# xuyuan/waymo_2d_tracking

Measured on AMD Instinct MI355X. Metric: end-to-end frames/sec (detect+SORT) on 1920x1280 Waymo frames, higher is better.
Workload: dtype f32; 1 GPU; Cascade R-CNN X152-32x8d-FPN dconv (random-init, fp32, batch 1) on synthetic 1920x1280x3 frames -> top-100 detections/frame -> SORT (max_age 2, min_hits 0, all boxes tracked; trackers resident for the whole segment); 5 cameras x 2 frames per step per GPU; 1x1 and dense 3x3 convolutions: f32 operands as exact 3 x bf16 splits, six cross terms on the bf16 matrix cores, f32 accumulate (csrc/det_gemm_s; stage=e2e, parallelism=sequence-shard x1

## Files before the change

include/waymodet.h:

```cpp
#ifndef WAYMODET_H
#define WAYMODET_H
#include <stddef.h>
#include <stdint.h>
#ifdef __cplusplus
extern "C" {
#endif

int wd_roi_pool_fpn_f32(const float* const* feats, const int32_t* heights, const int32_t* widths,
                        const float* scales, int n_levels, int channels, int batch,
                        const float* rois, int n_rois, int pooled, int min_level, int canonical_level,
                        float canonical_size, float* out, void* stream);

size_t wd_nms_workspace(int n);
int wd_select_kept(const uint8_t* keep_mask, const uint8_t* valid, const int64_t* order, int n, int cap, int64_t* out_idx,
                   int32_t* count, void* stream);
int wd_nms_sorted_f32(const float* boxes, const int32_t* idxs, int n, float iou_threshold,
                      uint8_t* keep_mask, int32_t* n_keep, void* workspace, size_t workspace_bytes, void* stream);

size_t wd_gemm_nt_workspace(int M, int N, int K);
int wd_gemm_nt_ws_f32(const float* A, const float* Bt, const float* bias, const float* residual, int relu, int M, int N, int K,
                      float* C, void* workspace, size_t workspace_bytes, void* stream);

int wd_gemm_lt_f32(const float* a, const float* w, const float* bias, const float* residual, float* out, int m, int n, int k,
                   int relu, void* workspace, size_t workspace_bytes, void* stream);
// ... 6 lines not shown
    void* dst;
    long s_n, s_c, s_kh, s_kw;
    long first_block;
    int N, K, C, ksize, flip, reserved;
} WdSplitPackDesc;
int wd_gemm_split_pack_batch(const WdSplitPackDesc* descs_device, int count, long total_blocks, void* stream);
size_t wd_gemm_split_workspace(long M, int N, int K);
int wd_gemm_split_f32(const float* a, long lda, const void* packed_w, const float* bias, const float* residual, float* out, long ldc,
                      int M, int N, int K, int relu, void* workspace, size_t workspace_bytes, void* stream);
int wd_conv_split_f32(const float* x, int batch, int H, int W, int C, const void* packed_w, int ksize, int stride, int pad, const float* bias,
                      const float* residual, float* out, int N, int relu, void* workspace, size_t workspace_bytes, void* stream);
int wd_gemm_split_supported(const float* a, long lda, const float* bias, const float* residual, const float* out, long ldc, long M, int N, int K);
int wd_conv_split_position_major(int batch, int H, int W, int ksize, int stride, int pad);
typedef struct WdSplitIO {
    const float* a;
    long lda;
    const void* a_planes;
    const float* residual;
    const void* residual_planes;
    float* out;
    void* out_planes;
    long ldc;
} WdSplitIO;
size_t wd_split_planes_bytes(long M, int K);
int wd_split_planes_pack_f32(const float* a, long lda, long M, int K, void* planes, void* stream);
int wd_split_planes_unpack_f32(const void* planes, long M, int K, float* out, long ldo, void* stream);
int wd_gemm_split_io(const WdSplitIO* io, const void* packed_w, const float* bias, int M, int N, int K, int relu, void* workspace,
                     size_t workspace_bytes, void* stream);
int wd_nms_segmented_f32(const float* boxes, const int32_t* idxs, const int32_t* seg_offsets, int n_seg, float iou_threshold,
                         uint8_t* keep_mask, int32_t* n_keep, void* workspace, size_t workspace_bytes, void* stream);

size_t wd_rpn_topk_workspace(const int* n_per_level, int n_levels, int k);
int wd_rpn_topk_decode_f32(const float* const* logits, const float* const* deltas, const float* const* anchors,
                           const int* n_per_level, int n_levels, int k, float img_h, float img_w, float scale_clamp,
                           float* out_boxes, float* out_scores, int32_t* out_group, uint8_t* out_valid, void* workspace,
                           size_t workspace_bytes, void* stream);
int wd_sort_candidates_f32(const float* boxes, const float* scores, const int32_t* group, const uint8_t* valid,
                           const uint8_t* valid2 , int n, float* out_boxes, float* out_scores, int32_t* out_group, uint8_t* out_valid, int64_t* out_order,
                           void* stream);
int wd_box_candidates_f32(const float* boxes, const float* s0, const float* s1, const float* s2, const int32_t* n_valid, int rows,
                          int num_classes, float score_thresh, float img_h, float img_w, float* out_boxes, float* out_scores,
                          int32_t* out_group, uint8_t* out_valid, int64_t* out_order, void* stream);
int wd_gather_kept_f32(const uint8_t* keep, const uint8_t* valid, const float* boxes, const float* scores, const int64_t* order,
                       int n, int cap, int num_classes, float* out_boxes, float* out_scores, int64_t* out_class, int32_t* count,
                       void* stream);
int wd_detections_to_wire(const float* boxes, const float* scores, const int64_t* classes, const int32_t* count, int n, int in_w,
                          int in_h, int hflip, int out_w, int out_h, double* xywhs, int32_t* category, void* stream);

size_t wd_deform_packed_weight_floats(int c_in, int c_out, int groups);
int wd_deform_pack_weight(const float* weight_oihw, int c_in, int c_out, int groups, float* packed, void* stream);
const char* wd_deform_conv3x3_variant(int c_in, int groups, int stride, int pad, int has_offset);
const char* wd_deform_conv3x3_last_kernel(void);
int wd_deform_conv3x3_f32(const float* x, const float* offset, const float* mask, const float* packed_weight,
                          const float* scale, const float* bias, int relu,
                          int batch, int h, int w, int c_in, int c_out, int groups, int stride, int pad,
                          float* y, void* stream);
int wd_deform_conv3x3_hint_f32(const float* x, const float* offset, const float* mask, const float* packed_weight,
                               const float* scale, const float* bias, int relu, int batch, int h, int w, int c_in,
                               int c_out, int groups, int stride, int pad, int far_offsets, float* y, void* stream);
size_t wd_deform_table_bytes(int batch, int h, int w);
int wd_deform_offsets_table_f32(const float* partial, int ld, const float* bias, int batch, int h, int w, float* offsets,
                                void* table, void* stream);
int wd_deform_conv3x3_tab_f32(const float* x, const float* offset, const float* mask, const float* packed_weight,
                              const float* scale, const float* bias, int relu, int batch, int h, int w, int c_in,
                              int c_out, int groups, int stride, int pad, int far_offsets, const void* table, float* y,
                              void* stream);

int wd_gemm_nt_f32(const float* A, const float* Bt, const float* bias, const float* residual, int relu,
                   int M, int N, int K, float* C, void* stream);

int wd_groupnorm_relu_nhwc_f32(float* x, const float* gamma, const float* beta, int n, int hw, int c, int groups,
                               float eps, int relu, void* stream);
int wd_groupnorm_relu_out_nhwc_f32(const float* x, float* y, const float* gamma, const float* beta, int n, int hw, int c, int groups,
                                   float eps, int relu, void* stream);
int wd_groupnorm_relu_bwd_nhwc_f32(const float* x, const float* dy, const float* gamma, const float* beta, int n, int hw, int c, int groups,
                                   float eps, int relu, float* dx, float* dgamma, float* dbeta, void* stream);

#define WD_LAYOUT_NCHW_F32 0
#define WD_LAYOUT_NHWC_U8 1
int wd_preprocess_out_shape(int h, int w, double scale, int divisor, int* ho, int* wo, int* hp, int* wp);
int wd_preprocess_f32(const void* src, int src_layout, int batch, int h, int w, double scale, int hflip, int vflip,
                      int swap_rb, const float* mean3, const float* std3, int divisor, float* out, void* stream);

int wd_decode_boxes_f32(const float* deltas, const float* boxes, const int64_t* index, int n, float wx, float wy, float ww,
                        float wh, float scale_clamp, float clip_w, float clip_h, float* out, void* stream);

int wd_roi_pool_fpn_bwd_f32(float* const* grad_feats, const int32_t* heights, const int32_t* widths, const float* scales,
                            int n_levels, int channels, int batch, const float* rois, int n_rois, int pooled, int min_level,
                            int canonical_level, float canonical_size, const float* grad_out, void* stream);
int wd_deform_im2col_f32(const float* x, const float* offset, int batch, int h, int w, int c, int groups, int stride, int pad,
                         float* col, void* stream);
int wd_deform_col2im_f32(const float* dcol, const float* x, const float* offset, int batch, int h, int w, int c, int groups,
                         int stride, int pad, float* dx, float* doffset, void* stream);
size_t wd_deform_bwd_tables_bytes(int batch, int h, int w, int stride);
int wd_deform_dxoff_f32(const float* x, const float* offset, const float* dy, const float* y_act, const float* scale, const float* weight, int batch,
                        int h, int w, int c, int groups, int stride, unsigned char* tables, float* packed_weight, float* dx, float* doffset,
                        void* stream);
size_t wd_deform_dw_scratch_floats(int batch, int h, int w, int c, int groups, int stride);
int wd_deform_dw_f32(const float* x, const float* offset, const float* dy, const float* y_act, const float* scale, int batch, int h, int w, int c,
                     int groups, int stride, float* scratch, float* dw, void* stream);

int wd_tap_shift_add_f32(const float* partial, int ld, int n_out, const float* bias, int batch, int h, int w, int stride,
                         float* out, void* stream);

int wd_upsample2x_nhwc_f32(const float* src, int batch, int h, int w, int c, float* dst, void* stream);

int wd_bias_relu_f32(float* y, const float* bias, long m, int n, int relu, void* stream);

int wd_act_bwd_f32(const float* dy, const float* y, const float* scale, long m, int n, int relu, float* g, void* stream);

int wd_autocontrast_u8(uint8_t* img, int h, int w, void* workspace24, void* stream);

int wd_jpeg_info(const uint8_t* data, int64_t n, int32_t* width, int32_t* height, int32_t* components, int32_t* h_samp,
                 int32_t* v_samp, int32_t* restart_interval);
int wd_jpeg_decode_rgb_u8(const uint8_t* data, int64_t n, uint8_t* rgb, int64_t capacity, int32_t* width, int32_t* height,
                          int32_t* sync_rounds, void* stream);
int wd_jpeg_last_stats(int32_t* out4);

#ifdef __cplusplus
}
#endif
#endif
```

waymo_2d_tracking_amd/build.py:

```python
import os
import subprocess
import sys
from concurrent.futures import ThreadPoolExecutor

HERE = os.path.dirname(os.path.abspath(__file__))
CSRC = os.path.join(HERE, 'csrc')
LIB = os.path.join(CSRC, 'libwaymotrack.so')
HIPCC = os.environ.get('HIPCC', '/opt/rocm/bin/hipcc')
ARCH = 'gfx950'

COMMON = ['--offload-arch=' + ARCH, '-O3', '-std=c++17', '-fPIC', '-fno-fast-math', '-Wall', '-Wno-unused-function']
COMMON += os.environ.get('WD_HIPCC_FLAGS', '').split()
UNITS = {
    'api.hip': [],
    'json_io.hip': [],
    'waymo_proto.hip': [],
    'ensemble.hip': ['-ffp-contract=off'],
    'ensemble_wbf.hip': ['-ffp-contract=off'],
    'sort_engine.hip': ['-ffp-contract=off'],
    'sort_single.hip': ['-ffp-contract=off'],
    'mot_eval.hip': ['-ffp-contract=off'],
    'mot_identity.hip': ['-ffp-contract=off'],
    'mot_hota.hip': ['-ffp-contract=off'],
    'track_refine.hip': ['-ffp-contract=off'],
    'det_eval.hip': ['-ffp-contract=off'],
    'det_roialign.hip': [],
    'det_nms.hip': [],
    'det_deform.hip': [],
    'det_deform_pp.hip': ['-fno-slp-vectorize'],
    'det_gconv.hip': [],
    'det_gemm.hip': ['-munsafe-fp-atomics'],
    'det_gemm_lt.hip': [],
    'det_gemm_split.hip': [],
    'det_misc.hip': [],
    'det_preprocess.hip': ['-ffp-contract=off'],
    'jpeg_decode.hip': [],
    'det_tail.hip': ['-ffp-contract=off'],
    'det_backward.hip': ['-munsafe-fp-atomics'],
    'det_deform_bwd.hip': ['-munsafe-fp-atomics'],
}
DEBUG_UNITS = {'det_gemm_split.hip': [], 'debug/debug_kernels.hip': []}
DEBUG_LIB = os.path.join(CSRC, 'libwaymotrack_debug.so')


def _newer(target, sources):
    if not os.path.exists(target):
        return True
    t = os.path.getmtime(target)
    return any(os.path.getmtime(s) > t for s in sources)


def build(force=False, verbose=True):
    headers = [os.path.join(CSRC, f) for f in os.listdir(CSRC) if f.endswith('.h')]
    headers += [os.path.join(HERE, '..', 'include', f) for f in os.listdir(os.path.join(HERE, '..', 'include'))]
    units = [u for u in UNITS if os.path.exists(os.path.join(CSRC, u))]
    objs = []
    jobs = []
    for u in units:
        src = os.path.join(CSRC, u)
        obj = os.path.join(CSRC, os.path.basename(u).replace('.hip', '.o'))
        objs.append(obj)
        if force or _newer(obj, [src] + headers):
            jobs.append([HIPCC] + COMMON + UNITS[u] + ['-c', src, '-o', obj])

    def run(cmd):
        if verbose:
            print(' '.join(cmd), flush=True)
        r = subprocess.run(cmd, capture_output=True, text=True)
        if r.returncode != 0:
            raise RuntimeError('hipcc failed:\n%s\n%s' % (' '.join(cmd), r.stderr[-6000:]))
        if verbose and r.stderr.strip():
            print(r.stderr[-3000:])
        return 0

    if jobs:
        with ThreadPoolExecutor(max_workers=min(6, len(jobs))) as ex:
            list(ex.map(run, jobs))
    if jobs or force or _newer(LIB, objs):
        run([HIPCC, '--offload-arch=' + ARCH, '-shared', '-fPIC', '-o', LIB] + objs)
    return LIB


def build_debug(force=False, verbose=True):
    build(force, verbose)
    headers = [os.path.join(CSRC, f) for f in os.listdir(CSRC) if f.endswith('.h')] + [os.path.join(CSRC, 'debug', 'waymodet_debug.h')]
    headers += [os.path.join(HERE, '..', 'include', f) for f in os.listdir(os.path.join(HERE, '..', 'include'))]
    objs = [os.path.join(CSRC, os.path.basename(u).replace('.hip', '.o')) for u in UNITS if u not in DEBUG_UNITS]
    jobs = []
    for u, flags in DEBUG_UNITS.items():
        src, obj = os.path.join(CSRC, u), os.path.join(CSRC, os.path.basename(u).replace('.hip', '.dbg.o'))
        objs.append(obj)
        if force or _newer(obj, [src] + headers):
            jobs.append([HIPCC] + COMMON + ['-DWD_DEBUG=1'] + UNITS.get(u, []) + flags + ['-c', src, '-o', obj])
    for cmd in jobs:
        if verbose:
            print(' '.join(cmd), flush=True)
        r = subprocess.run(cmd, capture_output=True, text=True)
        if r.returncode != 0:
            raise RuntimeError('hipcc failed:\n%s\n%s' % (' '.join(cmd), r.stderr[-6000:]))
    if jobs or force or _newer(DEBUG_LIB, objs):
        r = subprocess.run([HIPCC, '--offload-arch=' + ARCH, '-shared', '-fPIC', '-o', DEBUG_LIB] + objs, capture_output=True, text=True)
        if r.returncode != 0:
            raise RuntimeError('link failed:\n%s' % r.stderr[-6000:])
    return DEBUG_LIB


if __name__ == '__main__':
    if os.environ.get('WD_DEBUG_BUILD') == '1':
        print(build_debug(force='--force' in sys.argv))
    else:
        build(force='--force' in sys.argv)
    print(LIB)
```

waymo_2d_tracking_amd/detnet/nn/cascade_rcnn.py:

```python
import math
import os

import torch
from torch import nn
import torch.nn.functional as F

from . import ops

BLOCKS = (3, 8, 36, 3)
STAGE_CH = (256, 512, 1024, 2048)
GROUPS = 32
PIXEL_MEAN = (103.530, 116.280, 123.675)
PIXEL_STD = (57.375, 57.120, 58.395)
SCALE_CLAMP = math.log(1000.0 / 16)


FUSED_TRAINING_EPILOGUES = True


SPLIT_GEMM = os.environ.get('WD_SPLIT_GEMM', '1') != '0'


OFFSET_SPLIT_MIN_ROWS = 30000


SPLIT_PLANES = os.environ.get('WD_SPLIT_PLANES', '0') == '1'
SPLIT_PLANES_MIN_CH = int(os.environ.get('WD_SPLIT_PLANES_MIN_CH', '1024'))


class PlanesAct:

    def __init__(self, planes, n, h, w, c):
        self.planes, self.n, self.h, self.w, self.c = planes, n, h, w, c


DECISION_LOG = None


def _split_ok(cin, cout):
    return SPLIT_GEMM and cin % 64 == 0 and cout % 32 == 0


class _PackedSplit:

    def __init__(self):
        self.buf = None
        self.key = None

    def get(self, weight):
        key = (weight.device, weight._version, weight.data_ptr())
        if self.buf is None or self.key != key:
            self.buf = ops.split_pack_weight(weight)
            self.key = key
        return self.buf


def _msra(shape, gen, fan_out=True):
    w = torch.empty(shape)
    fan = shape[0] * shape[2] * shape[3] if fan_out else shape[1] * shape[2] * shape[3]
    return w.normal_(0, math.sqrt(2.0 / fan), generator=gen)


class Conv1x1(nn.Module):

    def __init__(self, cin, cout, gen, bn_scale=1.0, bias=False):
        super().__init__()
        w = _msra((cout, cin, 1, 1), gen).view(cout, cin)
        s = bn_scale / math.sqrt(1.0 + 1e-5) if not bias else 1.0
        self.weight = nn.Parameter(w * s, requires_grad=False)
        self.bias = nn.Parameter(torch.zeros(cout), requires_grad=False)
        self._split = _PackedSplit()

    def forward(self, x, relu=False, residual=None, stride=1):
        if not torch.is_grad_enabled() and x.is_cuda and _split_ok(self.weight.shape[1], self.weight.shape[0]):
            pw = self._split.get(self.weight)
            cout = self.weight.shape[0]
            if stride != 1 or not x.is_contiguous(memory_format=torch.channels_last):
                return ops.conv_split(x, pw, cout, 1, stride, 0, self.bias, residual, relu)
            n, c, h, w = x.shape
            a = x.permute(0, 2, 3, 1).reshape(n * h * w, c)
            r = None
            if residual is not None:
                r = residual if residual.is_contiguous(memory_format=torch.channels_last) else residual.contiguous(memory_format=torch.channels_last)
                r = r.permute(0, 2, 3, 1).reshape(n * h * w, cout)
            if ops.gemm_split_ok(a, cout, self.bias, r):
                y = ops.gemm_split(a, pw, cout, self.bias, r, relu, out=r)
                return y.view(n, h, w, cout).permute(0, 3, 1, 2)
        if stride != 1:
            x = x[:, :, ::stride, ::stride].contiguous(memory_format=torch.channels_last)
        n, c, h, w = x.shape
        a = x.permute(0, 2, 3, 1).reshape(n * h * w, c)
        r = None if residual is None else residual.permute(0, 2, 3, 1).reshape(n * h * w, -1)
        if torch.is_grad_enabled():
            if FUSED_TRAINING_EPILOGUES:
                y = ops.LinearActFn.apply(a, self.weight, self.bias, r, relu)
            else:
                y = F.linear(a, self.weight, self.bias)
                if r is not None:
                    y = y + r
                if relu:
                    y = F.relu(y)
            return y.view(n, h, w, -1).permute(0, 3, 1, 2)
        if r is None:
            if relu:
                y = torch._addmm_activation(self.bias, a, self.weight.t(), use_gelu=False)
            else:
                y = torch.addmm(self.bias, a, self.weight.t())
        else:
            if a.is_contiguous():
                y = ops.gemm_lt(a, self.weight, self.bias, r if r.is_contiguous() else r.contiguous(), relu,
                                out=r if r.is_contiguous() else None)
            else:
                y = r.addmm_(a, self.weight.t()) if r.is_contiguous() else torch.addmm(r, a, self.weight.t())
                y = ops.bias_relu_(y, self.bias, relu)
        return y.view(n, h, w, -1).permute(0, 3, 1, 2)


class ConvBN(nn.Module):

    def __init__(self, cin, cout, k, stride, pad, groups, gen, bias=False):
        super().__init__()
        w = _msra((cout, cin // groups, k, k), gen)
        s = 1.0 / math.sqrt(1.0 + 1e-5) if not bias else 1.0
        self.weight = nn.Parameter((w * s).contiguous(memory_format=torch.channels_last), requires_grad=False)
        self.bias = nn.Parameter(torch.zeros(cout), requires_grad=False)
        self.stride, self.pad, self.groups = stride, pad, groups
        self._split = _PackedSplit()

    def forward(self, x, relu=False):
        if (not torch.is_grad_enabled() and x.is_cuda and self.groups == 1 and self.weight.shape[2] in (1, 3)
                and _split_ok(self.weight.shape[1], self.weight.shape[0])):
            return ops.conv_split(x, self._split.get(self.weight), self.weight.shape[0], self.weight.shape[2], self.stride, self.pad,
                                  self.bias, None, relu)
        if not torch.is_grad_enabled() and self.weight.shape[0] % 4 == 0:
            y = F.conv2d(x, self.weight, None, self.stride, self.pad, 1, self.groups)
# ... 69 lines not shown
                out = ops.DeformConvFn.apply(out, offset, self.conv2_weight, GROUPS, self.stride, 1)
                out = F.relu(out * self.conv2_scale.view(1, -1, 1, 1) + self.conv2_bias.view(1, -1, 1, 1))
        elif self.deform:
            table = None
            if self.stride == 1 and self.conv2_weight.shape[1] in (16, 32):
                offset, table = self.offset_conv(out, deform_table=True)
            else:
                offset = self.offset_conv(out, stride=self.stride)
            out = ops.deform_conv3x3(out, offset, self.packed_weight(), GROUPS, self.stride, 1, self.conv2_scale,
                                     self.conv2_bias, relu=True, table=table)
        else:
            out = ops.deform_conv3x3(out, None, self.packed_weight(), GROUPS, self.stride, 1, self.conv2_scale,
                                     self.conv2_bias, relu=True)
        if rec is None:
            return self.conv3(out, relu=True, residual=sc)
        out3 = self.conv3(out, relu=True, residual=sc)
        rec.append((out1.detach().clone(), None if offset is None else offset.detach().clone(), out.detach().clone(), out3.detach().clone(), self.stride))
        return out3


def _bottleneck_forward_planes(self, x, emit_planes):
    in_planes = isinstance(x, PlanesAct)
    cout = self.conv3.weight.shape[0]
    if in_planes:
        assert self.shortcut is None and self.stride == 1
        n, h, w, cin = x.n, x.h, x.w, x.c
        m = n * h * w
        o1, _ = ops.gemm_split_io(m, self.conv1.weight.shape[0], cin, self.conv1._split.get(self.conv1.weight), a_planes=x.planes, bias=self.conv1.bias, relu=True)
        out = o1.view(n, h, w, -1).permute(0, 3, 1, 2)
        sc = None
    else:
        sc = x if self.shortcut is None else self.shortcut(x, stride=self.stride)
        out = self.conv1(x, relu=True)
    table = None
    if self.stride == 1 and self.conv2_weight.shape[1] in (16, 32):
        offset, table = self.offset_conv(out, deform_table=True)
    else:
        offset = self.offset_conv(out, stride=self.stride)
    out = ops.deform_conv3x3(out, offset, self.packed_weight(), GROUPS, self.stride, 1, self.conv2_scale, self.conv2_bias, relu=True, table=table)
    n, c, h, w = out.shape
    m = n * h * w
    a = out.permute(0, 2, 3, 1).reshape(m, c)
    pw = self.conv3._split.get(self.conv3.weight)
    if in_planes:
        y, yp = ops.gemm_split_io(m, cout, c, pw, a=a, bias=self.conv3.bias, residual_planes=x.planes, relu=True, want_out=not emit_planes,
                                  out_planes=x.planes if emit_planes else None, want_planes=False)
    else:
        r = sc if sc.is_contiguous(memory_format=torch.channels_last) else sc.contiguous(memory_format=torch.channels_last)
        r = r.permute(0, 2, 3, 1).reshape(m, cout)
        y, yp = ops.gemm_split_io(m, cout, c, pw, a=a, bias=self.conv3.bias, residual=r, relu=True, want_out=not emit_planes, want_planes=emit_planes)
    if emit_planes:
        return PlanesAct(yp, n, h, w, cout)
    return y.view(n, h, w, cout).permute(0, 3, 1, 2)


Bottleneck._forward_planes = _bottleneck_forward_planes


def _run_stage(stage, x):
    blocks = list(stage)
    use = (SPLIT_PLANES and SPLIT_GEMM and not torch.is_grad_enabled() and x.is_cuda and DECISION_LOG is None and len(blocks) > 1
           and blocks[0].conv3.weight.shape[0] >= SPLIT_PLANES_MIN_CH and blocks[0].deform)
    if not use:
        return stage(x)
    for i, blk in enumerate(blocks):
        x = blk(x, emit_planes=i + 1 < len(blocks))
    return x


class ResNeXt152FPN(nn.Module):
    def __init__(self, gen, offset_std=0.01):
        super().__init__()
        self.stem = ConvBN(3, 64, 7, 2, 3, 1, gen)
        stages = []
        cin = 64
        for si, (nb, cout) in enumerate(zip(BLOCKS, STAGE_CH)):
            blocks = []
            for b in range(nb):
                stride = 2 if (b == 0 and si > 0) else 1
                blocks.append(Bottleneck(cin, cout, stride, si > 0, gen, offset_std))
                cin = cout
            stages.append(nn.Sequential(*blocks))
        self.res2, self.res3, self.res4, self.res5 = stages
        self.lateral = nn.ModuleList([Conv1x1(c, 256, gen, bias=True) for c in STAGE_CH])
        self.output = nn.ModuleList([ConvBN(256, 256, 3, 1, 1, 1, gen, bias=True) for _ in STAGE_CH])

    def forward(self, x):
        return self.top_down(self.bottom_up(x))

    def bottom_up(self, x):
        with torch.no_grad():
            x = self.stem(x, relu=True)
            x = F.max_pool2d(x, kernel_size=3, stride=2, padding=1)
            c2 = self.res2(x)
        c3 = _run_stage(self.res3, c2); c4 = _run_stage(self.res4, c3); c5 = _run_stage(self.res5, c4)
        return [c2, c3, c4, c5]

    def top_down(self, feats):
        c5 = feats[3]
        prev = self.lateral[3](c5)
        outs = [self.output[3](prev)]
        for i in (2, 1, 0):
            if prev.is_cuda and not (torch.is_grad_enabled() and prev.requires_grad) and prev.shape[1] % 4 == 0:
                top = ops.upsample2x_nearest(prev)
            else:
                top = F.interpolate(prev, scale_factor=2.0, mode='nearest').contiguous(memory_format=torch.channels_last)
            prev = self.lateral[i](feats[i], residual=top)
            outs.insert(0, self.output[i](prev))
        p6 = F.max_pool2d(outs[3], kernel_size=1, stride=2, padding=0)
        return outs + [p6]


def apply_deltas(deltas, boxes, weights):
    wx, wy, ww, wh = weights
    widths = boxes[:, 2] - boxes[:, 0]
    heights = boxes[:, 3] - boxes[:, 1]
    ctr_x = boxes[:, 0] + 0.5 * widths
    ctr_y = boxes[:, 1] + 0.5 * heights
    dx = deltas[:, 0] / wx
    dy = deltas[:, 1] / wy
    dw = torch.clamp(deltas[:, 2] / ww, max=SCALE_CLAMP)
    dh = torch.clamp(deltas[:, 3] / wh, max=SCALE_CLAMP)
    pcx = dx * widths + ctr_x
    pcy = dy * heights + ctr_y
    pw = torch.exp(dw) * widths
    ph = torch.exp(dh) * heights
    return torch.stack((pcx - 0.5 * pw, pcy - 0.5 * ph, pcx + 0.5 * pw, pcy + 0.5 * ph), dim=1)


def clip_boxes(boxes, h, w):
    x1 = boxes[:, 0].clamp(min=0, max=w); y1 = boxes[:, 1].clamp(min=0, max=h)
    x2 = boxes[:, 2].clamp(min=0, max=w); y2 = boxes[:, 3].clamp(min=0, max=h)
    return torch.stack((x1, y1, x2, y2), dim=1)


class RPN(nn.Module):
    SIZES = (32, 64, 128, 256, 512)
    RATIOS = (0.5, 1.0, 2.0)
    STRIDES = (4, 8, 16, 32, 64)

    def __init__(self, gen, pre_nms_topk=1000, post_nms_topk=1000, nms_thresh=0.7):
        super().__init__()
        self.conv = ConvBN(256, 256, 3, 1, 1, 1, gen, bias=True)
        self.conv.weight.data.normal_(0, 0.01, generator=gen)
        self.objectness = Conv1x1(256, 3, gen, bias=True)
        self.objectness.weight.data.normal_(0, 0.01, generator=gen)
        self.deltas = Conv1x1(256, 12, gen, bias=True)
        self.deltas.weight.data.normal_(0, 0.01, generator=gen)
        self.pre, self.post, self.thr = pre_nms_topk, post_nms_topk, nms_thresh
        self._anchors = {}

    def anchors(self, level, h, w, device):
        key = (level, h, w, device)
        if key not in self._anchors:
            size, stride = self.SIZES[level], self.STRIDES[level]
            cell = []
            for r in self.RATIOS:
                aw = math.sqrt(size * size / r)
                ah = r * aw
                cell.append([-aw / 2, -ah / 2, aw / 2, ah / 2])
            cell = torch.tensor(cell, dtype=torch.float32, device=device)
            sx = torch.arange(0, w * stride, stride, dtype=torch.float32, device=device)
            sy = torch.arange(0, h * stride, stride, dtype=torch.float32, device=device)
            yy, xx = torch.meshgrid(sy, sx, indexing='ij')
            shifts = torch.stack((xx, yy, xx, yy), dim=-1).reshape(-1, 1, 4)
            self._anchors[key] = (shifts + cell.view(1, -1, 4)).reshape(-1, 4)
        return self._anchors[key]

    def _level_ids(self, level, k, device):
        key = (level, k, device)
        if key not in self._anchors:
            self._anchors[key] = torch.full((k,), level, dtype=torch.int32, device=device)
        return self._anchors[key]

    def forward(self, feats, img_h, img_w):
        logits_l, deltas_l, anchors_l = [], [], []
        for l, f in enumerate(feats):
            t = self.conv(f, relu=True)
            logits = self.objectness(t)
            deltas = self.deltas(t)
            logits_l.append(logits.permute(0, 2, 3, 1).reshape(-1))
            deltas_l.append(deltas.permute(0, 2, 3, 1).reshape(-1, 4))
            anchors_l.append(self.anchors(l, f.shape[2], f.shape[3], f.device))
        boxes, scores, lvls, ok = ops.rpn_topk_decode(logits_l, deltas_l, anchors_l, self.pre, img_h, img_w)
        seg = [0]
        for lg in logits_l:
            seg.append(seg[-1] + min(self.pre, lg.numel()))
        keep = ops.nms_segmented(boxes, lvls, seg, self.thr)
        sb, ss, sg, sv, order = ops.sort_candidates(boxes, scores, lvls, ok, keep)
        props, count = ops.gather_kept(sv, sv, sb, ss, order, self.post)
        return props, count


class BoxHead(nn.Module):

    def __init__(self, num_classes, gen):
        super().__init__()
        self.convs = nn.ModuleList([nn.Conv2d(256, 256, 3, 1, 1, bias=False) for _ in range(4)])
        self.norms = nn.ModuleList([nn.GroupNorm(32, 256) for _ in range(4)])
        for c in self.convs:
            c.weight.data.copy_(_msra((256, 256, 3, 3), gen))
        self.fc1_weight = nn.Parameter(torch.empty(1024, 12544).normal_(0, math.sqrt(1.0 / 12544), generator=gen),
                                       requires_grad=False)
        self.fc1_bias = nn.Parameter(torch.zeros(1024), requires_grad=False)
        self.cls_weight = nn.Parameter(torch.empty(num_classes + 1, 1024).normal_(0, 0.01, generator=gen), requires_grad=False)
        self.cls_bias = nn.Parameter(torch.zeros(num_classes + 1), requires_grad=False)
        self.box_weight = nn.Parameter(torch.empty(4, 1024).normal_(0, 0.001, generator=gen), requires_grad=False)
        self.box_bias = nn.Parameter(torch.zeros(4), requires_grad=False)
        self._split = [_PackedSplit() for _ in range(4)]
        self._split_fc = _PackedSplit()

    def forward(self, x):
        train = torch.is_grad_enabled()
        for li, (conv, norm) in enumerate(zip(self.convs, self.norms)):
            if not train and x.is_cuda and _split_ok(256, 256):
                x = ops.conv_split(x, self._split[li].get(conv.weight), 256, 3, 1, 1)
            elif train and ops.SPLIT_TRAIN and x.is_cuda and _split_ok(256, 256) and x.shape[0] > 0:
                x = ops.ConvSplitFn.apply(x, conv.weight, None, 1, 1, False)
            else:
                x = conv(x)
            if train:
                if FUSED_TRAINING_EPILOGUES and x.shape[2] * x.shape[3] <= 64 and x.shape[0] > 0:
                    x = ops.GroupNormReluFn.apply(x, norm.weight, norm.bias, norm.num_groups, norm.eps, True)
                else:
                    x = F.relu(norm(x))
                continue
            if not x.is_contiguous(memory_format=torch.channels_last):
                x = x.contiguous(memory_format=torch.channels_last)
            x = ops.groupnorm_relu_(x, norm.weight, norm.bias, norm.num_groups, norm.eps, True)
        r = x.shape[0]
        flat = x.permute(0, 2, 3, 1).reshape(r, -1)
        if train:
            h = F.relu(F.linear(flat, self.fc1_weight, self.fc1_bias))
        elif x.is_cuda and _split_ok(self.fc1_weight.shape[1], self.fc1_weight.shape[0]):
            h = ops.gemm_split(flat if flat.is_contiguous() else flat.contiguous(), self._split_fc.get(self.fc1_weight), self.fc1_weight.shape[0],
                               self.fc1_bias, None, True)
        else:
            h = ops.gemm_nt(flat, self.fc1_weight, self.fc1_bias, None, True)
        nc1 = self.cls_weight.shape[0]
        if not train and x.is_cuda and nc1 + 4 <= 32 and _split_ok(1024, 32):
            key = (self.cls_weight._version, self.box_weight._version, self.cls_bias._version, self.box_bias._version, self.cls_weight.device)
            if getattr(self, '_pred_key', None) != key:
                wcat = torch.zeros(32, 1024, device=h.device)
                wcat[:nc1] = self.cls_weight.detach()
                wcat[nc1:nc1 + 4] = self.box_weight.detach()
                bcat = torch.zeros(32, device=h.device)
                bcat[:nc1] = self.cls_bias.detach()
                bcat[nc1:nc1 + 4] = self.box_bias.detach()
                self._pred_packed, self._pred_bias, self._pred_key = ops.split_pack_weight(wcat), bcat, key
            out = ops.gemm_split(h, self._pred_packed, 32, self._pred_bias, None, False)
            return out[:, :nc1], out[:, nc1:nc1 + 4]
        logits = F.linear(h, self.cls_weight, self.cls_bias)
        deltas = F.linear(h, self.box_weight, self.box_bias)
        return logits, deltas


class CascadeRCNN(nn.Module):
    CASCADE_WEIGHTS = ((10.0, 10.0, 5.0, 5.0), (20.0, 20.0, 10.0, 10.0), (30.0, 30.0, 15.0, 15.0))

    def __init__(self, num_classes=4, seed=0, score_thresh=0.01, nms_thresh=0.5, topk=100, offset_std=0.01):
        super().__init__()
        gen = torch.Generator().manual_seed(seed)
        self.num_classes = num_classes
        self.backbone = ResNeXt152FPN(gen, offset_std)
        self.rpn = RPN(gen)
        self.heads = nn.ModuleList([BoxHead(num_classes, gen) for _ in range(3)])
# ... 88 lines not shown
```

waymo_2d_tracking_amd/detnet/nn/ops.py:

```python
import ctypes as C
import os

import torch

from ... import _lib


EVENT_LOG = None


_RAW_STREAM = getattr(torch._C, '_cuda_getCurrentRawStream', None)
_RAW_DEVICE = getattr(torch._C, '_cuda_getDevice', None)


def _stream():
    if _RAW_STREAM is not None and _RAW_DEVICE is not None:
        return C.c_void_p(_RAW_STREAM(_RAW_DEVICE()))
    return C.c_void_p(torch.cuda.current_stream().cuda_stream)


def _p(t):
    return C.c_void_p(t.data_ptr()) if t is not None else None


# ... 462 lines not shown
def split_planes_bytes(m, k):
    return int(_lib.lib().wd_split_planes_bytes(C.c_long(m), C.c_int(k)))


def split_planes_empty(m, k, device):
    n = split_planes_bytes(m, k)
    if n == 0:
        raise ValueError('activation planes need K %% 32 == 0 (M=%d K=%d)' % (m, k))
    return torch.empty(n, dtype=torch.uint8, device=device)


def split_planes_pack(a, out=None):
    m, k = a.shape
    assert a.dtype == torch.float32 and a.stride(1) == 1
    if out is None:
        out = split_planes_empty(m, k, a.device)
    _lib.check(_lib.lib().wd_split_planes_pack_f32(_p(a), C.c_long(a.stride(0)), C.c_long(m), C.c_int(k), _p(out), _stream()), 'wd_split_planes_pack_f32')
    return out


def split_planes_unpack(planes, m, k):
    out = torch.empty((m, k), dtype=torch.float32, device=planes.device)
    _lib.check(_lib.lib().wd_split_planes_unpack_f32(_p(planes), C.c_long(m), C.c_int(k), _p(out), C.c_long(k), _stream()), 'wd_split_planes_unpack_f32')
    return out


def gemm_split_io(m, n, k, packed, a=None, a_planes=None, bias=None, residual=None, residual_planes=None, relu=False, out=None, out_planes=None,
                  want_out=True, want_planes=False):
    dev = packed.device
    if want_out and out is None:
        out = torch.empty((m, n), dtype=torch.float32, device=dev)
    if want_planes and out_planes is None:
        out_planes = split_planes_empty(m, n, dev)
    io = _SplitIO()
    if a is not None:
        assert a.dtype == torch.float32 and a.stride(1) == 1 and tuple(a.shape) == (m, k)
        io.a, io.lda = a.data_ptr(), a.stride(0)
    if a_planes is not None:
        io.a_planes = a_planes.data_ptr()
    if residual is not None:
        assert residual.is_contiguous()
        io.residual = residual.data_ptr()
    if residual_planes is not None:
        io.residual_planes = residual_planes.data_ptr()
    if out is not None:
        assert out.is_contiguous()
        io.out = out.data_ptr()
    if out_planes is not None:
        io.out_planes = out_planes.data_ptr()
    io.ldc = n
    ws, ws_bytes = _split_workspace(m, n, k, dev)
    ev = _split_log_begin()
    _lib.check(_lib.lib().wd_gemm_split_io(C.byref(io), _p(packed), _p(bias), C.c_int(m), C.c_int(n), C.c_int(k), C.c_int(1 if relu else 0), _p(ws),
                                           C.c_size_t(ws_bytes), _stream()), 'wd_gemm_split_io')
    _split_log_end(ev, '%s: 1x1 conv / GEMM M=%d N=%d K=%d' % ('gemm_split_planes_kernel' if a_planes is not None else 'gemm_split_kernel', m, n, k), m, n, k)
    return out, out_planes


def conv_split(x, packed, n_out, ksize, stride=1, pad=0, bias=None, residual=None, relu=False):
    x = _nhwc(x)
    b, c, h, w = x.shape
    ho, wo = (h + 2 * pad - ksize) // stride + 1, (w + 2 * pad - ksize) // stride + 1
    out = torch.empty((b, n_out, ho, wo), dtype=torch.float32, device=x.device, memory_format=torch.channels_last)
    if _DEBUG_FILL:
        out.fill_(float('nan'))
    if residual is not None:
        residual = _nhwc(residual)
    ws, ws_bytes = _split_workspace(b * ho * wo, n_out, ksize * ksize * c, x.device)
    ev = _split_log_begin()
    _lib.check(_lib.lib().wd_conv_split_f32(_p(x), C.c_int(b), C.c_int(h), C.c_int(w), C.c_int(c), _p(packed), C.c_int(ksize), C.c_int(stride),
                                            C.c_int(pad), _p(bias), _p(residual), _p(out), C.c_int(n_out), C.c_int(1 if relu else 0), _p(ws), C.c_size_t(ws_bytes),
                                            _stream()),
               'wd_conv_split_f32')
    if ev is not None:
        k_eff = ksize * ksize * c
        if _lib.lib().wd_conv_split_position_major(C.c_int(b), C.c_int(h), C.c_int(w), C.c_int(ksize), C.c_int(stride), C.c_int(pad)):
            walked = (h - 2) * (w - 2) * 9 + (2 * (h - 2) + 2 * (w - 2)) * 6 + 4 * 4
            k_eff = k_eff * walked / float(9 * h * w)
        _split_log_end(ev, 'gemm_split_kernel: %dx%d conv s%d M=%d N=%d K=%d' % (ksize, ksize, stride, b * ho * wo, n_out, ksize * ksize * c), b * ho * wo,
                       n_out, k_eff)
    return out


SCALE_CLAMP = 4.135166556742356


def _ptr_array(tensors):
    return (C.c_void_p * len(tensors))(*[t.data_ptr() for t in tensors])


def rpn_topk_decode(logits, deltas, anchors, k, img_h, img_w):
    logits = [t.contiguous().float() for t in logits]
    deltas = [t.contiguous().float() for t in deltas]
    anchors = [t.contiguous().float() for t in anchors]
    n = [int(t.numel()) for t in logits]
    dev = logits[0].device
    rows = sum(min(k, v) for v in n)
    counts = (C.c_int * len(n))(*n)
    lib = _lib.lib()
    need = int(lib.wd_rpn_topk_workspace(counts, C.c_int(len(n)), C.c_int(k)))
    ws = torch.empty(need, dtype=torch.uint8, device=dev)
    boxes = torch.empty((rows, 4), dtype=torch.float32, device=dev)
    scores = torch.empty(rows, dtype=torch.float32, device=dev)
    group = torch.empty(rows, dtype=torch.int32, device=dev)
    valid = torch.empty(rows, dtype=torch.uint8, device=dev)
    _lib.check(lib.wd_rpn_topk_decode_f32(_ptr_array(logits), _ptr_array(deltas), _ptr_array(anchors), counts, C.c_int(len(n)),
                                          C.c_int(k), C.c_float(img_h), C.c_float(img_w), C.c_float(SCALE_CLAMP), _p(boxes),
                                          _p(scores), _p(group), _p(valid), _p(ws), C.c_size_t(need), _stream()),
               'wd_rpn_topk_decode_f32')
    return boxes, scores, group, valid


def _sorted_outputs(n, dev):
    return (torch.empty((n, 4), dtype=torch.float32, device=dev), torch.empty(n, dtype=torch.float32, device=dev),
            torch.empty(n, dtype=torch.int32, device=dev), torch.empty(n, dtype=torch.uint8, device=dev),
            torch.empty(n, dtype=torch.int64, device=dev))


def sort_candidates(boxes, scores, group, valid, valid2=None):
    n = boxes.shape[0]
    out = _sorted_outputs(n, boxes.device)
    _lib.check(_lib.lib().wd_sort_candidates_f32(_p(boxes), _p(scores), _p(group), _p(valid), _p(valid2), C.c_int(n),
                                                 *[_p(t) for t in out], _stream()), 'wd_sort_candidates_f32')
    return out


def nms_segmented(boxes, idxs, seg_offsets, iou_threshold, return_count=False):
    n = boxes.shape[0]
    keep = torch.zeros(n, dtype=torch.uint8, device=boxes.device)
    if n == 0:
        return (keep, torch.zeros(len(seg_offsets) - 1, dtype=torch.int32, device=boxes.device)) if return_count else keep
    lib = _lib.lib()
    need = int(lib.wd_nms_workspace(C.c_int(n)))
    key = (boxes.device, torch.cuda.current_stream().cuda_stream)
    ws = _nms_ws.get(key)
    if ws is None or ws.numel() < need:
        ws = torch.empty(need, dtype=torch.uint8, device=boxes.device)
        _nms_ws[key] = ws
    n_seg = len(seg_offsets) - 1
    cnt = torch.zeros(n_seg, dtype=torch.int32, device=boxes.device)
    offs = (C.c_int32 * (n_seg + 1))(*[int(v) for v in seg_offsets])
    _lib.check(lib.wd_nms_segmented_f32(_p(boxes.contiguous()), _p(idxs), offs, C.c_int(n_seg), C.c_float(iou_threshold), _p(keep),
                                        _p(cnt), _p(ws), C.c_size_t(ws.numel()), _stream()), 'wd_nms_segmented_f32')
    return (keep, cnt) if return_count else keep


def box_candidates(boxes, s0, s1, s2, n_valid, score_thresh, img_h, img_w):
    r, nc = s0.shape[0], s0.shape[1] - 1
    out = _sorted_outputs(r * nc, boxes.device)
    _lib.check(_lib.lib().wd_box_candidates_f32(_p(boxes.contiguous()), _p(s0.contiguous()), _p(s1.contiguous()), _p(s2.contiguous()),
                                                _p(n_valid), C.c_int(r), C.c_int(nc), C.c_float(score_thresh), C.c_float(img_h),
                                                C.c_float(img_w), *[_p(t) for t in out], _stream()), 'wd_box_candidates_f32')
    return out


def gather_kept(keep, valid, boxes, scores, order, cap, num_classes=0):
    dev = boxes.device
    ob = torch.empty((cap, 4), dtype=torch.float32, device=dev)
    cnt = torch.empty(1, dtype=torch.int32, device=dev)
    if num_classes:
        osc = torch.empty(cap, dtype=torch.float32, device=dev)
        oc = torch.empty(cap, dtype=torch.int64, device=dev)
    else:
        osc = oc = None
    _lib.check(_lib.lib().wd_gather_kept_f32(_p(keep), _p(valid), _p(boxes), _p(scores), _p(order), C.c_int(boxes.shape[0]),
                                             C.c_int(cap), C.c_int(num_classes), _p(ob), _p(osc), _p(oc), _p(cnt), _stream()),
# ... 322 lines not shown
```

Baseline: 44.91 frames/s.

## Fuse stem conv+ReLU+maxpool and batch RPN 1x1 predictors into single kernels

Adds a fused stem kernel that computes the 7x7 stride-2 conv on fp32 MFMA, applies bias and ReLU, and does the 3x3 stride-2 maxpool from a shared-memory tile. This avoids writing and re-reading the full-resolution stem activation. It also adds one persistent kernel that evaluates the RPN objectness and delta 1x1 heads for all FPN levels in a single launch, replacing many small per-level GEMMs and permutes. Both paths are gated to inference with fp32 and standard shapes. The stem uses plain fp32 MFMA rather than the split-bf16 path, which may change numerics slightly.

```diff
diff --git a/include/waymodet.h b/include/waymodet.h
--- a/include/waymodet.h
+++ b/include/waymodet.h
@@ -112,6 +112,16 @@
 int wd_preprocess_f32(const void* src, int src_layout, int batch, int h, int w, double scale, int hflip, int vflip,
                       int swap_rb, const float* mean3, const float* std3, int divisor, float* out, void* stream);
 
+int wd_stem_pack_weight_f32(const float* weight, float* packed, void* stream);
+int wd_stem_fused_f32(const float* x, int n, int h, int w, const float* packed, const float* bias, float* out, void* stream);
+
+typedef struct WdRpnLevels {
+    const float* hidden[8];
+    long pixels[8];
+    int n_levels;
+} WdRpnLevels;
+int wd_rpn_predict_f32(const WdRpnLevels* levels, const float* weight, const float* bias, float* out_logits, float* out_deltas, void* stream);
+
 int wd_decode_boxes_f32(const float* deltas, const float* boxes, const int64_t* index, int n, float wx, float wy, float ww,
                         float wh, float scale_clamp, float clip_w, float clip_h, float* out, void* stream);
 
diff --git a/waymo_2d_tracking_amd/build.py b/waymo_2d_tracking_amd/build.py
--- a/waymo_2d_tracking_amd/build.py
+++ b/waymo_2d_tracking_amd/build.py
@@ -34,6 +34,8 @@
     'det_gemm_split.hip': [],
     'det_misc.hip': [],
     'det_preprocess.hip': ['-ffp-contract=off'],
+    'det_stem.hip': [],
+    'det_rpn_predict.hip': [],
     'jpeg_decode.hip': [],
     'det_tail.hip': ['-ffp-contract=off'],
     'det_backward.hip': ['-munsafe-fp-atomics'],
diff --git a/waymo_2d_tracking_amd/csrc/det_rpn_predict.hip b/waymo_2d_tracking_amd/csrc/det_rpn_predict.hip
--- /dev/null
+++ b/waymo_2d_tracking_amd/csrc/det_rpn_predict.hip
@@ -0,0 +1,144 @@
+#include "common.h"
+#include "../../include/waymodet.h"
+
+namespace {
+
+typedef float f32x2 __attribute__((ext_vector_type(2)));
+
+constexpr int kK = 256;
+constexpr int kOut = 15;
+constexpr int kPairs = 8;
+constexpr int kPix = 4;
+constexpr int kRows = kPix * 4;
+constexpr int kLd = 68;
+constexpr int kWaves = 4;
+constexpr int kMaxLevels = 8;
+
+struct Levels {
+    const float* x[kMaxLevels];
+    long first[kMaxLevels + 1];
+    int n_levels;
+};
+
+__device__ __forceinline__ float quad_xor1(float v) {
+    return __builtin_bit_cast(float, __builtin_amdgcn_mov_dpp(__builtin_bit_cast(int, v), 0xB1, 0xF, 0xF, true));
+}
+__device__ __forceinline__ float quad_xor2(float v) {
+    return __builtin_bit_cast(float, __builtin_amdgcn_mov_dpp(__builtin_bit_cast(int, v), 0x4E, 0xF, 0xF, true));
+}
+
+__global__ __launch_bounds__(kWaves * 64) void rpn_predict_kernel(const Levels lv, const float* __restrict__ weight, const float* __restrict__ bias,
+                                                                 float* __restrict__ logits, float* __restrict__ deltas) {
+    __shared__ float part_all[kWaves][kRows * kLd];
+    const int lane = threadIdx.x & 63;
+    const int wave = threadIdx.x >> 6;
+    float* part = part_all[wave];
+    const long total = lv.first[lv.n_levels];
+    const long steps = (total + kPix - 1) / kPix;
+
+    f32x2 w2[kPairs][4];
+#pragma unroll
+    for (int i = 0; i < kPairs; ++i) {
+        const float4 wa = reinterpret_cast<const float4*>(weight + (2 * i) * kK)[lane];
+        float4 wb = make_float4(0.f, 0.f, 0.f, 0.f);
+        if (2 * i + 1 < kOut) wb = reinterpret_cast<const float4*>(weight + (2 * i + 1) * kK)[lane];
+        w2[i][0] = f32x2{wa.x, wb.x}; w2[i][1] = f32x2{wa.y, wb.y}; w2[i][2] = f32x2{wa.z, wb.z}; w2[i][3] = f32x2{wa.w, wb.w};
+    }
+    const bool odd1 = lane & 1, odd2 = lane & 2;
+    const int my_pix = lane >> 4, my_col = lane & 15;
+    const float my_bias = my_col < kOut ? bias[my_col] : 0.f;
+    const float* my_row = part + (lane >> 2) * kLd + (lane & 3);
+
+    auto load = [&](long step, float4 (&x)[kPix]) {
+#pragma unroll
+        for (int j = 0; j < kPix; ++j) {
+            const long p = step * kPix + j;
+            x[j] = make_float4(0.f, 0.f, 0.f, 0.f);
+            if (p < total) {
+                int l = 0;
+                while (l + 1 < lv.n_levels && p >= lv.first[l + 1]) ++l;
+                x[j] = reinterpret_cast<const float4*>(lv.x[l] + (p - lv.first[l]) * kK)[lane];
+            }
+        }
+    };
+    const long stride = (long)gridDim.x * kWaves;
+    long step = (long)blockIdx.x * kWaves + wave;
+    float4 x[kPix], xn[kPix];
+    if (step < steps) load(step, xn);
+    for (; step < steps; step += stride) {
+        const long p0 = step * kPix;
+#pragma unroll
+        for (int j = 0; j < kPix; ++j) x[j] = xn[j];
+        if (step + stride < steps) load(step + stride, xn);
+#pragma unroll
+        for (int j = 0; j < kPix; ++j)
+#pragma unroll
+            for (int g = 0; g < 4; ++g) {
+                f32x2 s[2];
+#pragma unroll
+                for (int h = 0; h < 2; ++h) {
+                    s[h] = w2[2 * g + h][0] * x[j].x;
+                    s[h] = w2[2 * g + h][1] * x[j].y + s[h];
+                    s[h] = w2[2 * g + h][2] * x[j].z + s[h];
+                    s[h] = w2[2 * g + h][3] * x[j].w + s[h];
+                }
+                const float k0 = (odd1 ? s[0].y : s[0].x) + quad_xor1(odd1 ? s[0].x : s[0].y);
+                const float k1 = (odd1 ? s[1].y : s[1].x) + quad_xor1(odd1 ? s[1].x : s[1].y);
+                const float r = (odd2 ? k1 : k0) + quad_xor2(odd2 ? k0 : k1);
+                part[(j * 4 + g) * kLd + lane] = r;
+            }
+        __builtin_amdgcn_fence(__ATOMIC_RELEASE, "wavefront");
+        __builtin_amdgcn_wave_barrier();
+        __builtin_amdgcn_fence(__ATOMIC_ACQUIRE, "wavefront");
+        {
+            float a[4];
+#pragma unroll
+            for (int c = 0; c < 4; ++c) a[c] = my_row[4 * c];
+#pragma unroll
+            for (int q = 4; q < 16; ++q) a[q & 3] += my_row[4 * q];
+            const float sum = ((a[0] + a[1]) + (a[2] + a[3])) + my_bias;
+            const long p = p0 + my_pix;
+            if (p < total && my_col < kOut) {
+                if (my_col < 3) logits[p * 3 + my_col] = sum;
+                else deltas[p * 12 + (my_col - 3)] = sum;
+            }
+        }
+        __builtin_amdgcn_fence(__ATOMIC_RELEASE, "wavefront");
+        __builtin_amdgcn_wave_barrier();
+        __builtin_amdgcn_fence(__ATOMIC_ACQUIRE, "wavefront");
+    }
+}
+
+}
+
+extern "C" int wd_rpn_predict_f32(const WdRpnLevels* levels, const float* weight, const float* bias, float* out_logits, float* out_deltas,
+                                  void* stream) {
+    WT_TRY(wt::ensure_device());
+    if (!levels || levels->n_levels < 1 || levels->n_levels > kMaxLevels || !weight || !bias || !out_logits || !out_deltas ||
+        ((uintptr_t)weight & 15)) {
+        wt::set_error("wd_rpn_predict_f32: bad argument (1..%d levels, weight 16-byte aligned)", kMaxLevels);
+        return WT_ERR_INVALID;
+    }
+    Levels lv;
+    memset(&lv, 0, sizeof(lv));
+    lv.n_levels = levels->n_levels;
+    long total = 0;
+    for (int l = 0; l < lv.n_levels; ++l) {
+        if (!levels->hidden[l] || levels->pixels[l] < 1 || ((uintptr_t)levels->hidden[l] & 15)) {
+            wt::set_error("wd_rpn_predict_f32: level %d is empty or its map is not 16-byte aligned", l);
+            return WT_ERR_INVALID;
+        }
+        lv.x[l] = levels->hidden[l];
+        lv.first[l] = total;
+        total += levels->pixels[l];
+    }
+    lv.first[lv.n_levels] = total;
+    const long steps = (total + kPix - 1) / kPix;
+    long blocks = (steps + kWaves - 1) / kWaves;
+    const long cap = 4L * (wt::device_cus() > 0 ? wt::device_cus() : 256);
+    if (blocks > cap) blocks = cap;
+    hipLaunchKernelGGL(rpn_predict_kernel, dim3((unsigned)blocks), dim3(kWaves * 64), 0, (hipStream_t)stream, lv, weight, bias, out_logits,
+                       out_deltas);
+    WT_HIP(hipGetLastError());
+    return WT_OK;
+}
diff --git a/waymo_2d_tracking_amd/csrc/det_stem.hip b/waymo_2d_tracking_amd/csrc/det_stem.hip
--- /dev/null
+++ b/waymo_2d_tracking_amd/csrc/det_stem.hip
@@ -0,0 +1,181 @@
+#include "common.h"
+#include "../../include/waymodet.h"
+
+namespace {
+
+typedef float f32x4 __attribute__((ext_vector_type(4)));
+
+constexpr int kCout = 64;
+constexpr int kTaps = 147;
+constexpr int kSteps = 37;
+constexpr int kTileY = 4, kTileX = 8;
+constexpr int kConvY = 2 * kTileY + 1;
+constexpr int kConvX = 2 * kTileX + 1;
+constexpr int kM = kConvY * kConvX;
+constexpr int kMTiles = (kM + 15) / 16;
+constexpr int kPatchY = 2 * (kConvY - 1) + 7;
+constexpr int kPatchX = 2 * (kConvX - 1) + 7;
+constexpr int kPatchLd = kPatchX * 3;
+constexpr int kPatch = kPatchY * kPatchLd;
+constexpr int kStageLd = kCout + 4;
+constexpr int kThreads = 256;
+constexpr int kPatchRegs = (kPatch + kThreads - 1) / kThreads;
+static_assert(kMTiles % 2 == 0, "the k loop carries two accumulators");
+
+__global__ void stem_pack_kernel(const float* __restrict__ w, float* __restrict__ packed) {
+    const int i = blockIdx.x * blockDim.x + threadIdx.x;
+    if (i >= kSteps * 4 * kCout) return;
+    const int k = i / kCout, o = i - k * kCout;
+    packed[i] = k < kTaps ? w[o * kTaps + k] : 0.f;
+}
+
+__global__ __launch_bounds__(kThreads, 3) void stem_fused_kernel(const float* __restrict__ x, int n, int h, int w, const float* __restrict__ packed,
+                                                              const float* __restrict__ bias, float* __restrict__ out, int hc, int wc, int hp, int wp,
+                                                              int tiles_x, int tiles_y) {
+    __shared__ float patch[kPatch + 1];
+    __shared__ __attribute__((aligned(16))) float stage[kM * kStageLd];
+    const int tid = threadIdx.x;
+    const int lane = tid & 63, wave = tid >> 6;
+    const int col = lane & 15, kq = lane >> 4;
+
+    float wreg[kSteps];
+#pragma unroll
+    for (int s = 0; s < kSteps; ++s) wreg[s] = packed[(4 * s + kq) * kCout + 16 * wave + col];
+    f32x4 b4 = {0.f, 0.f, 0.f, 0.f};
+    if (bias) b4 = *reinterpret_cast<const f32x4*>(bias + 16 * wave + 4 * kq);
+
+    const long tiles = (long)n * tiles_y * tiles_x;
+    float pre[kPatchRegs];
+    auto fetch = [&](long tile) {
+        const int tx = (int)(tile % tiles_x);
+        const int ty = (int)((tile / tiles_x) % tiles_y);
+        const int img = (int)(tile / ((long)tiles_x * tiles_y));
+        const int iy0 = 4 * ty * kTileY - 5, ix0 = 4 * tx * kTileX - 5;
+        const float* img_x = x + (long)img * h * w * 3;
+#pragma unroll
+        for (int e = 0; e < kPatchRegs; ++e) {
+            const int i = tid + e * kThreads;
+            const int r = i / kPatchLd, q = i - r * kPatchLd;
+            const int gy = iy0 + r, gq = ix0 * 3 + q;
+            float v = 0.f;
+            if (i < kPatch && gy >= 0 && gy < h && gq >= 0 && gq < w * 3) v = img_x[((long)gy * w) * 3 + gq];
+            pre[e] = v;
+        }
+    };
+    if ((long)blockIdx.x < tiles) fetch(blockIdx.x);
+    for (long tile = blockIdx.x; tile < tiles; tile += gridDim.x) {
+        const int tx = (int)(tile % tiles_x);
+        const int ty = (int)((tile / tiles_x) % tiles_y);
+        const int img = (int)(tile / ((long)tiles_x * tiles_y));
+        const int py0 = ty * kTileY, px0 = tx * kTileX;
+        const int cy0 = 2 * py0 - 1, cx0 = 2 * px0 - 1;
+#pragma unroll
+        for (int e = 0; e < kPatchRegs; ++e) {
+            const int i = tid + e * kThreads;
+            if (i < kPatch) patch[i] = pre[e];
+        }
+        __syncthreads();
+        if (tile + gridDim.x < tiles) fetch(tile + gridDim.x);
+
+#pragma unroll 1
+        for (int mp = 0; mp < kMTiles / 2; ++mp) {
+            int m0 = 32 * mp + col, m1 = m0 + 16;
+            const bool live0 = m0 < kM, live1 = m1 < kM;
+            if (!live0) m0 = kM - 1;
+            if (!live1) m1 = kM - 1;
+            const int base0 = (m0 / kConvX) * (2 * kPatchLd) + (m0 % kConvX) * 6;
+            const int base1 = (m1 / kConvX) * (2 * kPatchLd) + (m1 % kConvX) * 6;
+            f32x4 acc0[4], acc1[4];
+#pragma unroll
+            for (int c = 0; c < 4; ++c) {
+                acc0[c] = f32x4{0.f, 0.f, 0.f, 0.f};
+                acc1[c] = f32x4{0.f, 0.f, 0.f, 0.f};
+            }
+            int adr0[4], adr1[4];
+#pragma unroll
+            for (int v = 0; v < 4; ++v) {
+                const int wrap = kq >= 4 - v ? kPatchLd - 21 : 0;
+                adr0[v] = base0 + kq + wrap;
+                adr1[v] = base1 + kq + wrap;
+            }
+#pragma unroll
+            for (int s = 0; s < kSteps; ++s) {
+                const int r = (4 * s) % 21, q = (4 * s) / 21;
+                const int v = (s == kSteps - 1 || r <= 17) ? 0 : r - 17;
+                float a0 = patch[adr0[v] + q * kPatchLd + r];
+                float a1 = patch[adr1[v] + q * kPatchLd + r];
+                if (s == kSteps - 1 && kq == 3) { a0 = 0.f; a1 = 0.f; }
+                acc0[s & 3] = __builtin_amdgcn_mfma_f32_16x16x4f32(wreg[s], a0, acc0[s & 3], 0, 0, 0);
+                acc1[s & 3] = __builtin_amdgcn_mfma_f32_16x16x4f32(wreg[s], a1, acc1[s & 3], 0, 0, 0);
+            }
+            if (live0) {
+                f32x4 v = ((acc0[0] + acc0[1]) + (acc0[2] + acc0[3])) + b4;
+                v.x = fmaxf(v.x, 0.f); v.y = fmaxf(v.y, 0.f); v.z = fmaxf(v.z, 0.f); v.w = fmaxf(v.w, 0.f);
+                *reinterpret_cast<f32x4*>(stage + m0 * kStageLd + 16 * wave + 4 * kq) = v;
+            }
+            if (live1) {
+                f32x4 v = ((acc1[0] + acc1[1]) + (acc1[2] + acc1[3])) + b4;
+                v.x = fmaxf(v.x, 0.f); v.y = fmaxf(v.y, 0.f); v.z = fmaxf(v.z, 0.f); v.w = fmaxf(v.w, 0.f);
+                *reinterpret_cast<f32x4*>(stage + m1 * kStageLd + 16 * wave + 4 * kq) = v;
+            }
+        }
+        __syncthreads();
+
+#pragma unroll
+        for (int it = 0; it < kTileY * kTileX * (kCout / 4) / kThreads; ++it) {
+            const int item = tid + it * kThreads;
+            const int cq = item & 15, pp = item >> 4;
+            const int ppy = pp / kTileX, ppx = pp % kTileX;
+            const int py = py0 + ppy, px = px0 + ppx;
+            if (py < hp && px < wp) {
+                f32x4 best = *reinterpret_cast<const f32x4*>(stage + ((2 * ppy + 1) * kConvX + 2 * ppx + 1) * kStageLd + 4 * cq);
+#pragma unroll
+                for (int dy = 0; dy < 3; ++dy) {
+                    const int cy = cy0 + 2 * ppy + dy;
+                    if (cy < 0 || cy >= hc) continue;
+#pragma unroll
+                    for (int dx = 0; dx < 3; ++dx) {
+                        const int cx = cx0 + 2 * ppx + dx;
+                        if (cx < 0 || cx >= wc || (dy == 1 && dx == 1)) continue;
+                        const f32x4 v = *reinterpret_cast<const f32x4*>(stage + ((2 * ppy + dy) * kConvX + 2 * ppx + dx) * kStageLd + 4 * cq);
+                        best.x = fmaxf(best.x, v.x); best.y = fmaxf(best.y, v.y); best.z = fmaxf(best.z, v.z); best.w = fmaxf(best.w, v.w);
+                    }
+                }
+                *reinterpret_cast<f32x4*>(out + (((long)img * hp + py) * wp + px) * kCout + 4 * cq) = best;
+            }
+        }
+    }
+}
+
+}
+
+extern "C" int wd_stem_pack_weight_f32(const float* weight, float* packed, void* stream) {
+    WT_TRY(wt::ensure_device());
+    if (!weight || !packed) {
+        wt::set_error("wd_stem_pack_weight_f32: null pointer");
+        return WT_ERR_INVALID;
+    }
+    const int total = kSteps * 4 * kCout;
+    hipLaunchKernelGGL(stem_pack_kernel, dim3((total + 255) / 256), dim3(256), 0, (hipStream_t)stream, weight, packed);
+    WT_HIP(hipGetLastError());
+    return WT_OK;
+}
+
+extern "C" int wd_stem_fused_f32(const float* x, int n, int h, int w, const float* packed, const float* bias, float* out, void* stream) {
+    WT_TRY(wt::ensure_device());
+    if (n <= 0 || h <= 0 || w <= 0) return WT_OK;
+    if (!x || !packed || !out || ((uintptr_t)out & 15) || (bias && ((uintptr_t)bias & 15)) || (long)h * w * 3 > 0x7fffffffL) {
+        wt::set_error("wd_stem_fused_f32: bad argument (out and bias 16-byte aligned, h * w * 3 < 2^31)");
+        return WT_ERR_INVALID;
+    }
+    const int hc = (h - 1) / 2 + 1, wc = (w - 1) / 2 + 1;
+    const int hp = (hc - 1) / 2 + 1, wp = (wc - 1) / 2 + 1;
+    const int tiles_y = (hp + kTileY - 1) / kTileY, tiles_x = (wp + kTileX - 1) / kTileX;
+    const long tiles = (long)n * tiles_y * tiles_x;
+    long blocks = 3L * (wt::device_cus() > 0 ? wt::device_cus() : 256);
+    if (blocks > tiles) blocks = tiles;
+    hipLaunchKernelGGL(stem_fused_kernel, dim3((unsigned)blocks), dim3(kThreads), 0, (hipStream_t)stream, x, n, h, w, packed, bias, out, hc, wc,
+                       hp, wp, tiles_x, tiles_y);
+    WT_HIP(hipGetLastError());
+    return WT_OK;
+}
diff --git a/waymo_2d_tracking_amd/detnet/nn/cascade_rcnn.py b/waymo_2d_tracking_amd/detnet/nn/cascade_rcnn.py
--- a/waymo_2d_tracking_amd/detnet/nn/cascade_rcnn.py
+++ b/waymo_2d_tracking_amd/detnet/nn/cascade_rcnn.py
@@ -43,14 +43,15 @@
 
 class _PackedSplit:
 
-    def __init__(self):
+    def __init__(self, pack=None):
         self.buf = None
         self.key = None
+        self.pack = pack or ops.split_pack_weight
 
     def get(self, weight):
         key = (weight.device, weight._version, weight.data_ptr())
         if self.buf is None or self.key != key:
-            self.buf = ops.split_pack_weight(weight)
+            self.buf = self.pack(weight)
             self.key = key
         return self.buf
 
@@ -286,6 +287,7 @@
                 cin = cout
             stages.append(nn.Sequential(*blocks))
         self.res2, self.res3, self.res4, self.res5 = stages
+        self._stem_packed = _PackedSplit(ops.stem_pack_weight)
         self.lateral = nn.ModuleList([Conv1x1(c, 256, gen, bias=True) for c in STAGE_CH])
         self.output = nn.ModuleList([ConvBN(256, 256, 3, 1, 1, 1, gen, bias=True) for _ in STAGE_CH])
 
@@ -293,12 +295,21 @@
         return self.top_down(self.bottom_up(x))
 
     def bottom_up(self, x):
+        fused_stem = not torch.is_grad_enabled() and x.is_cuda and x.dtype == torch.float32 and self._stem_is_standard()
         with torch.no_grad():
-            x = self.stem(x, relu=True)
-            x = F.max_pool2d(x, kernel_size=3, stride=2, padding=1)
+            if fused_stem:
+                x = ops.stem_fused(x, self._stem_packed.get(self.stem.weight), self.stem.bias)
+            else:
+                x = self.stem(x, relu=True)
+                x = F.max_pool2d(x, kernel_size=3, stride=2, padding=1)
             c2 = self.res2(x)
         c3 = _run_stage(self.res3, c2); c4 = _run_stage(self.res4, c3); c5 = _run_stage(self.res5, c4)
         return [c2, c3, c4, c5]
+
+    def _stem_is_standard(self):
+        st = self.stem
+        return (tuple(st.weight.shape) == (64, 3, 7, 7) and st.stride == 2 and st.pad == 3 and st.groups == 1
+                and st.weight.dtype == torch.float32 and st.bias.dtype == torch.float32)
 
     def top_down(self, feats):
         c5 = feats[3]
@@ -377,15 +388,28 @@
             self._anchors[key] = torch.full((k,), level, dtype=torch.int32, device=device)
         return self._anchors[key]
 
+    def _pred_packed(self):
+        ps = (self.objectness.weight, self.deltas.weight, self.objectness.bias, self.deltas.bias)
+        key = (ps[0].device,) + tuple(p._version for p in ps) + tuple(p.data_ptr() for p in ps)
+        if getattr(self, '_pred_key', None) != key:
+            self._pred_w = torch.cat((ps[0].detach(), ps[1].detach()), 0).float().contiguous()
+            self._pred_b = torch.cat((ps[2].detach(), ps[3].detach()), 0).float().contiguous()
+            self._pred_key = key
+        return self._pred_w, self._pred_b
+
     def forward(self, feats, img_h, img_w):
-        logits_l, deltas_l, anchors_l = [], [], []
-        for l, f in enumerate(feats):
-            t = self.conv(f, relu=True)
-            logits = self.objectness(t)
-            deltas = self.deltas(t)
-            logits_l.append(logits.permute(0, 2, 3, 1).reshape(-1))
-            deltas_l.append(deltas.permute(0, 2, 3, 1).reshape(-1, 4))
-            anchors_l.append(self.anchors(l, f.shape[2], f.shape[3], f.device))
+        anchors_l = [self.anchors(l, f.shape[2], f.shape[3], f.device) for l, f in enumerate(feats)]
+        if (not torch.is_grad_enabled() and len(feats) <= 8 and all(f.is_cuda and f.dtype == torch.float32 and f.shape[0] == 1 for f in feats)
+                and tuple(self.objectness.weight.shape) == (3, 256) and tuple(self.deltas.weight.shape) == (12, 256)):
+            logits_l, deltas_l = ops.rpn_predict([self.conv(f, relu=True) for f in feats], *self._pred_packed())
+        else:
+            logits_l, deltas_l = [], []
+            for f in feats:
+                t = self.conv(f, relu=True)
+                logits = self.objectness(t)
+                deltas = self.deltas(t)
+                logits_l.append(logits.permute(0, 2, 3, 1).reshape(-1))
+                deltas_l.append(deltas.permute(0, 2, 3, 1).reshape(-1, 4))
         boxes, scores, lvls, ok = ops.rpn_topk_decode(logits_l, deltas_l, anchors_l, self.pre, img_h, img_w)
         seg = [0]
         for lg in logits_l:
diff --git a/waymo_2d_tracking_amd/detnet/nn/ops.py b/waymo_2d_tracking_amd/detnet/nn/ops.py
--- a/waymo_2d_tracking_amd/detnet/nn/ops.py
+++ b/waymo_2d_tracking_amd/detnet/nn/ops.py
@@ -568,6 +568,56 @@
     return out
 
 
+def stem_pack_weight(weight):
+    assert tuple(weight.shape) == (64, 3, 7, 7) and weight.is_cuda
+    w = weight.detach().float().permute(0, 2, 3, 1).contiguous()
+    packed = torch.empty((148, 64), dtype=torch.float32, device=weight.device)
+    _lib.check(_lib.lib().wd_stem_pack_weight_f32(_p(w), _p(packed), _stream()), 'wd_stem_pack_weight_f32')
+    return packed
+
+
+def stem_out_shape(h, w):
+    hc, wc = (h - 1) // 2 + 1, (w - 1) // 2 + 1
+    return (hc - 1) // 2 + 1, (wc - 1) // 2 + 1
+
+
+def stem_fused(x, packed, bias):
+    x = _nhwc(x)
+    n, c, h, w = x.shape
+    assert c == 3
+    hp, wp = stem_out_shape(h, w)
+    out = torch.empty((n, 64, hp, wp), dtype=torch.float32, device=x.device, memory_format=torch.channels_last)
+    _lib.check(_lib.lib().wd_stem_fused_f32(_p(x), C.c_int(n), C.c_int(h), C.c_int(w), _p(packed), _p(bias), _p(out), _stream()),
+               'wd_stem_fused_f32')
+    return out
+
+
+class _RpnLevels(C.Structure):
+    _fields_ = [('hidden', C.c_void_p * 8), ('pixels', C.c_long * 8), ('n_levels', C.c_int)]
+
+
+def rpn_predict(hidden, weight, bias):
+    assert 1 <= len(hidden) <= 8 and tuple(weight.shape) == (15, 256) and weight.is_contiguous()
+    hidden = [_nhwc(t) for t in hidden]
+    desc = _RpnLevels()
+    desc.n_levels = len(hidden)
+    pix = []
+    for l, t in enumerate(hidden):
+        assert t.shape[1] == 256
+        pix.append(t.shape[0] * t.shape[2] * t.shape[3])
+        desc.hidden[l] = t.data_ptr()
+        desc.pixels[l] = pix[-1]
+    total = sum(pix)
+    dev = hidden[0].device
+    logits = torch.empty(total * 3, dtype=torch.float32, device=dev)
+    deltas = torch.empty((total * 3, 4), dtype=torch.float32, device=dev)
+    _lib.check(_lib.lib().wd_rpn_predict_f32(C.byref(desc), _p(weight), _p(bias), _p(logits), _p(deltas), _stream()), 'wd_rpn_predict_f32')
+    lo = [0]
+    for v in pix:
+        lo.append(lo[-1] + 3 * v)
+    return [logits[lo[l]:lo[l + 1]] for l in range(len(pix))], [deltas[lo[l]:lo[l + 1]] for l in range(len(pix))]
+
+
 SCALE_CLAMP = 4.135166556742356
 
 
```

New measurement: 45.03 frames/s, median of 5. No clear change (+0.3%).
